# younggyoseo/CaDM

Measured on AMD Instinct MI355X. Metric: CEM rollout row-steps/s (cand x part x horizon x 5 CEM iters per get_action; ens=5 members), higher is better.
Workload: dtype f32 (each fp32 product as 3 f16 MFMA products of 2-way split operands, fp32 accumulate; error <= 2^-22 per product; measured parity: see `parity`); 1 GPU; cfg2: halfcheetah PE-TS+CaDM get_action, ens=5 part=20 cand=200 (200/GPU) H=30 m=1, random-init weights; global_candidates=200, parallelism=candidate-shard x1, collective=none, rccl_nranks=1

## Files before the change

### cadm_amd/csrc/pack_xdl.hip

```cpp
#include "common.h"
#include "xdl_geo.h"

namespace {

struct XdlPackArgs {
    const float* W[CADM_MAX_HIDDEN_LAYERS + 2];
    const float* b[CADM_MAX_HIDDEN_LAYERS + 2];
    unsigned short* dst;
    float* bias;
    int* overflow;
    XdlGeo g;
    int E;
    int swish_fold;
};

__device__ __forceinline__ unsigned short f16_bits(_Float16 h) { return __builtin_bit_cast(unsigned short, h); }

__global__ void pack_xdl_kernel(const XdlPackArgs a) {
    const XdlGeo& g = a.g;
    const size_t per_member = (size_t)g.member_frags() * 1024;
    const size_t total = per_member * a.E;
    for (size_t idx = blockIdx.x * (size_t)blockDim.x + threadIdx.x; idx < total; idx += (size_t)gridDim.x * blockDim.x) {
        const int e = idx / per_member;
        size_t rem = idx % per_member;
        int w = 0;
        while (rem >= (size_t)g.wave_frags(w) * 1024) { rem -= (size_t)g.wave_frags(w) * 1024; ++w; }
        int fj = rem / 1024;
        const int part = (rem % 1024) / 512;
        const int lane = (rem % 512) / 8;
        const int i = rem % 8;
        const int ntw = g.ntw(w);
        int layer, nchl;
        const int nc0s = g.NC0 - g.INV;
        const int inv0 = ntw * nc0s + (g.NH - 1) * ntw * g.NCH + g.nhead(w) * g.NCH;
        bool invf = false;
        if (g.INV && fj >= inv0) { invf = true; layer = 0; nchl = 1; fj -= inv0; }
        else if (fj < ntw * nc0s) { layer = 0; nchl = nc0s; }
        else {
            fj -= ntw * nc0s;
            layer = 1 + fj / (ntw * g.NCH);
            nchl = g.NCH;
            if (layer < g.NH) fj -= (layer - 1) * ntw * g.NCH;
            else { fj -= (g.NH - 1) * ntw * g.NCH; layer = g.NH; }
        }
        const int grp = lane >> 4, m = lane & 15;
        int tile, c;
        if (invf) { tile = g.tstart(w) + fj; c = g.NC0 - 1; }
        else if (layer < g.NH) {
            const int gsz = xdl_group();
            const int gi = fj / (gsz * nchl), jj = fj - gsz * gi * nchl;
            const int gs = (ntw - gsz * gi) < gsz ? (ntw - gsz * gi) : gsz;
            c = jj / gs;
            tile = g.tstart(w) + gsz * gi + jj % gs;
        } else {
            int sv = fj / g.NCH;
            c = fj % g.NCH;
            tile = -1;
            for (int s = 0; s < g.NTOW; ++s) {
                if (g.head_tile(w, s) < g.NTO) { if (sv == 0) { tile = g.head_tile(w, s); break; } --sv; }
            }
        }
        int kin;
        if (layer == 0) { kin = 32 * c + 8 * grp + i; if (kin >= g.K0) kin = -1; }
        else { kin = (2 * c + (i >> 2)) * 16 + 4 * grp + (i & 3); if (kin >= g.HIDR) kin = -1; }
        const int K = layer == 0 ? g.K0 : g.HIDR;
        float v = 0.0f;
        if (kin >= 0 && tile >= 0) {
            if (layer < g.NH) {
                const int u = 16 * tile + m;
                if (u < g.HIDR) v = a.W[layer][((size_t)e * K + kin) * g.HIDR + u];
            } else {
                const int q = m >> 2, r = m & 3;
                const int d = 8 * tile + 2 * q + (r & 1);
                if (d < g.D) v = a.W[g.NH + (r >> 1)][((size_t)e * K + kin) * g.D + d];
            }
        }
        if (a.swish_fold) v *= layer == 0 ? CADM_XDL_LOG2E : layer == g.NH ? (1.0f / CADM_XDL_LOG2E) : 1.0f;
        if (!(fabsf(v) <= 65000.0f)) { *a.overflow = 1; v = 0.0f; }
        const _Float16 v1 = (_Float16)v;
        const _Float16 v2 = (_Float16)((v - (float)v1) * 2048.0f);
        a.dst[idx] = f16_bits(part == 0 ? v1 : v2);
    }
}

__global__ void pack_xdl_bias_kernel(const XdlPackArgs a) {
    const XdlGeo& g = a.g;
    const size_t per = (size_t)g.bias_tiles() * 256;
    const size_t total = per * a.E;
    for (size_t idx = blockIdx.x * (size_t)blockDim.x + threadIdx.x; idx < total; idx += (size_t)gridDim.x * blockDim.x) {
        const int e = idx / per;
        const size_t rem = idx % per;
        int tile = rem / 256;
        const int lane = (rem % 256) / 4, r = rem % 4, grp = lane >> 4;
        float v = 0.0f;
        if (tile < g.NH * g.NT) {
            const int layer = tile / g.NT;
            tile %= g.NT;
            const int u = 16 * tile + 4 * grp + r;
            if (u < g.HIDR) v = a.b[layer][(size_t)e * g.HIDR + u];
            if (a.swish_fold) v *= CADM_XDL_LOG2E;
        } else {
            tile -= g.NH * g.NT;
            const int d = 8 * tile + 2 * grp + (r & 1);
            if (d < g.D) v = a.b[g.NH + (r >> 1)][(size_t)e * g.D + d];
// ... 41 lines not shown
```

### cadm_amd/csrc/rollout_xdl.h

```cpp
#pragma once
#include "rollout_args.h"
#include "rollout_env.h"
#include "xdl_geo.h"

namespace {

typedef _Float16 f16x8 __attribute__((ext_vector_type(8)));
typedef _Float16 f16x4 __attribute__((ext_vector_type(4)));
typedef _Float16 f16x2 __attribute__((ext_vector_type(2)));
typedef float floatx2 __attribute__((ext_vector_type(2)));

template <int ENV_, int C_, int HID_, int MT_, int NH_, int ACT_>
struct XC {
    static constexpr int ENV = ENV_, C = C_, HID = HID_, MT = MT_, NHC = NH_, ACT = ACT_;
    static_assert(NH_ >= 1 && NH_ <= CADM_MAX_HIDDEN_LAYERS, "number of hidden layers");
    static constexpr int D = env_D(ENV), A = env_A(ENV), P = env_P(ENV);
    static constexpr int K0 = P + A + C;
    static constexpr int NC0 = (K0 + 31) / 32;
    static constexpr bool SPARE = (K0 % 32) != 0;
    static constexpr int NT = (HID + 15) / 16;
    static constexpr bool INV = xdl_inv0(K0, P + A, HID);
    static constexpr int NC0S = NC0 - (INV ? 1 : 0);
    static constexpr int NCH = (NT + 1) / 2;
    static constexpr int NTO = (D + 7) / 8;
    static constexpr int NW = CADM_XDL_WAVES, NTHR = NW * 64;
    static constexpr int BASE = NT / NW, EXTRA = NT % NW;
    static constexpr int NTOW = (NTO + NW - 1) / NW;
    static_assert(NTOW == 1, "one head tile per wave at most (obs dim <= 64)");
    static constexpr int R = 4;
    static constexpr int NPROD = HID > 256 ? 4 : 3;
    static constexpr int NP = (D + 1) / 2, NPI = (NP + 15) / 16, NAI = (A + 15) / 16;
    static_assert(BASE >= 1, "hidden width too small for the 8-wave tile split (>= 128)");
    static constexpr int XIN = 0;
    static constexpr int XIN_T = 2 * NC0 * 1024, ACT_T = 2 * NCH * 1024, OFULL_T = NTO * 1024;
    static constexpr int ACTA = XIN + MT * XIN_T;
    static constexpr int ACTB = ACTA + MT * ACT_T;
    static constexpr int OFULL = ACTB + MT * ACT_T;
    static constexpr int STATS = OFULL + MT * OFULL_T;
    static constexpr int ST_OBS_MEAN = 0, ST_OBS_DEN = P, ST_ACT_MEAN = 2 * P, ST_ACT_DEN = 2 * P + A;
    static constexpr int TABW = 28;
    static constexpr int TAB = STATS + rup((2 * P + 2 * A) * 4, 16);
    static constexpr bool ONED = MT == 1 && NPI == 1 && D + NP <= 32 && A <= D;
    static constexpr int TABD = 16;
    static constexpr int TAB_BYTES = ONED ? 32 * TABD * 4 : NPI * 16 * TABW * 4;
    static constexpr int ZB = TAB + TAB_BYTES;
    static constexpr int ZB_T = 2 * NPI * 256 * 8;
    static constexpr int CTRL = ZB + MT * ZB_T;
    static constexpr int RES_1 = 16;
    static constexpr int RES_MT2_LESS = 6;
// ... 41 lines not shown

__device__ __forceinline__ void xres_load(uintx4& dst, __amdgpu_buffer_rsrc_t rsrc, unsigned voff, unsigned soff) {
    asm volatile("s_nop 4\n\tbuffer_load_dwordx4 %0, %1, %2, %3 offen"
                 : "=a"(dst) : "v"(voff), "s"(rsrc), "s"(__builtin_amdgcn_readfirstlane(soff)) : "memory");
}
__device__ __forceinline__ void xmfma_res(floatx4& acc, const uintx4& w, const f16x8& x) {
    asm volatile("s_nop 1\n\tv_mfma_f32_16x16x32_f16 %0, %1, %2, %0" : "+v"(acc) : "a"(w), "v"(x));
}
template <bool ASM>
__device__ __forceinline__ void xmfma_ring(floatx4& acc, const uintx4& w, const f16x8& x) {
    if constexpr (ASM) asm volatile("s_nop 1\n\tv_mfma_f32_16x16x32_f16 %0, %1, %2, %0" : "+v"(acc) : "v"(w), "v"(x));
    else acc = xmfma(w, x, acc);
}
template <bool LL>
__device__ __forceinline__ void xdl_result_nops(floatx4& a, floatx4& b, floatx4& c) {
    if constexpr (LL) asm volatile("s_nop 7\n\ts_nop 7\n\ts_nop 3" : "+v"(a), "+v"(b), "+v"(c));
    else asm volatile("s_nop 7\n\ts_nop 7\n\ts_nop 3" : "+v"(a), "+v"(b));
}
template <bool LL>
__device__ __forceinline__ void xdl_operand_nops(floatx4& a, floatx4& b, floatx4& c) {
    if constexpr (LL) asm volatile("s_nop 4" : "+v"(a), "+v"(b), "+v"(c));
    else asm volatile("s_nop 4" : "+v"(a), "+v"(b));
}

__device__ __forceinline__ void xsplit(float v, _Float16& hi, _Float16& lo) {
    hi = (_Float16)v;
    lo = (_Float16)(v - (float)hi);
}

template <class G, bool PACKED = true>
struct XHiddenEpi {
    static constexpr int NSTAGE = 6;
    struct StateP { floatx2 v[2], s[2]; f16x4 h1, h2; };
    struct StateS { float v[4], s[4]; f16x4 h1, h2; };
    using State = std::conditional_t<PACKED, StateP, StateS>;
    unsigned char* xsmem;
    const float* xb;
    int bias_off;
    int layer, out, tstart, lane;
    const unsigned char* inv = nullptr;
    __device__ __forceinline__ floatx4 init(int ti, int hh) const {
        if (inv) return *reinterpret_cast<const floatx4*>(inv + ((hh * G::NT + tstart + ti) * 2 + 0) * 1024 + lane * 16);
        const int tile = layer * G::NT + tstart + ti;
        const int bt = tile * 64 + lane;
        if constexpr (G::BIAS_LDS) return *reinterpret_cast<const floatx4*>(xsmem + bias_off + tile * G::BIAS_TILE_B + (lane >> 4) * 16);
        else return *reinterpret_cast<const floatx4*>(xb + bt * 4);
    }
    __device__ __forceinline__ floatx4 init_lo(int ti, int hh) const {
        if (inv) return *reinterpret_cast<const floatx4*>(inv + ((hh * G::NT + tstart + ti) * 2 + 1) * 1024 + lane * 16);
        return floatx4{0.f, 0.f, 0.f, 0.f};
    }
    static __device__ __forceinline__ floatx2 lo2(const floatx4& x) { return __builtin_shufflevector(x, x, 0, 1); }
    static __device__ __forceinline__ floatx2 hi2(const floatx4& x) { return __builtin_shufflevector(x, x, 2, 3); }
    template <int S>
    __device__ __forceinline__ void stage(int ti, int hh, const floatx4& hi, const floatx4& lo, const floatx4& ll, State& st) const {
        constexpr float KE = G::ACT == CADM_ACT_TANH ? -2.0f * 1.4426950408889634f : -1.4426950408889634f;
        constexpr bool SIG = G::ACT != CADM_ACT_RELU && G::ACT != CADM_ACT_NONE;
        if constexpr (PACKED) {
        if constexpr (S == 0) {
            const floatx2 c11 = {4.8828125e-4f, 4.8828125e-4f};
            const floatx2 ke = {KE, KE};
#pragma unroll
            for (int q = 0; q < 2; ++q) {
                const floatx2 pre = __builtin_elementwise_fma(q ? hi2(lo) : lo2(lo), c11, q ? hi2(hi) : lo2(hi));
                st.v[q] = pre;
                if constexpr (G::ACT == CADM_ACT_SWISH) st.s[q] = -pre;
                else st.s[q] = pre * ke;
            }
        } else if constexpr (S == 1) {
            if constexpr (SIG) {
#pragma unroll
                for (int q = 0; q < 2; ++q) { st.s[q][0] = __builtin_amdgcn_exp2f(st.s[q][0]); st.s[q][1] = __builtin_amdgcn_exp2f(st.s[q][1]); }
            }
        } else if constexpr (S == 2) {
            if constexpr (SIG) {
                const floatx2 one = {1.0f, 1.0f};
#pragma unroll
                for (int q = 0; q < 2; ++q) {
                    st.s[q] = st.s[q] + one;
                    st.s[q][0] = __builtin_amdgcn_rcpf(st.s[q][0]);
                    st.s[q][1] = __builtin_amdgcn_rcpf(st.s[q][1]);
                }
            }
        } else if constexpr (S == 3) {
#pragma unroll
            for (int q = 0; q < 2; ++q) {
                if constexpr (G::ACT == CADM_ACT_SWISH) st.v[q] = st.v[q] * st.s[q];
                else if constexpr (G::ACT == CADM_ACT_SIGMOID) st.v[q] = st.s[q];
                else if constexpr (G::ACT == CADM_ACT_TANH) {
#pragma unroll
                    for (int r = 0; r < 2; ++r) {
                        const float x = st.v[q][r], x2 = x * x;
                        const float ser = x * fmaf(x2, fmaf(x2, fmaf(x2, -0.05396825396825397f, 0.13333333333333333f), -0.3333333333333333f), 1.0f);
                        st.v[q][r] = fabsf(x) < 0.1f ? ser : fmaf(2.0f, st.s[q][r], -1.0f);
                    }
                } else if constexpr (G::ACT == CADM_ACT_RELU) { st.v[q][0] = fmaxf(st.v[q][0], 0.0f); st.v[q][1] = fmaxf(st.v[q][1], 0.0f); }
                st.h1[2 * q] = (_Float16)st.v[q][0];
                st.h1[2 * q + 1] = (_Float16)st.v[q][1];
            }
        } else if constexpr (S == 4) {
#pragma unroll
            for (int q = 0; q < 2; ++q) {
                const floatx2 t = st.v[q];
                const f16x2 hp = {st.h1[2 * q], st.h1[2 * q + 1]};
                f16x2 lp;
                asm("v_fma_mixlo_f16 %0, %1, %2, %3 op_sel_hi:[1,0,0]\n\tv_fma_mixhi_f16 %0, %1, %2, %4 op_sel:[1,0,0] op_sel_hi:[1,0,0]"
                    : "=&v"(lp) : "v"(hp), "s"(-1.0f), "v"(t[0]), "v"(t[1]));
                st.h2[2 * q] = lp[0];
                st.h2[2 * q + 1] = lp[1];
            }
        }
        } else {
        if constexpr (S == 0) {
#pragma unroll
            for (int r = 0; r < 4; ++r) {
                st.v[r] = fmaf(lo[r], 4.8828125e-4f, hi[r]);
                if constexpr (SIG && G::ACT != CADM_ACT_SWISH) st.s[r] = st.v[r] * KE;
            }
        } else if constexpr (S == 1) {
            if constexpr (SIG) {
#pragma unroll
                for (int r = 0; r < 4; ++r) st.s[r] = __builtin_amdgcn_exp2f(G::ACT == CADM_ACT_SWISH ? -st.v[r] : st.s[r]);
            }
        } else if constexpr (S == 2) {
            if constexpr (SIG) {
// ... 5 lines not shown
            for (int r = 0; r < 4; ++r) {
                if constexpr (G::ACT == CADM_ACT_SWISH) st.v[r] = st.v[r] * st.s[r];
                else if constexpr (G::ACT == CADM_ACT_SIGMOID) st.v[r] = st.s[r];
                else if constexpr (G::ACT == CADM_ACT_TANH) {
                    const float x = st.v[r], x2 = x * x;
                    const float ser = x * fmaf(x2, fmaf(x2, fmaf(x2, -0.05396825396825397f, 0.13333333333333333f), -0.3333333333333333f), 1.0f);
                    st.v[r] = fabsf(x) < 0.1f ? ser : fmaf(2.0f, st.s[r], -1.0f);
                } else if constexpr (G::ACT == CADM_ACT_RELU) st.v[r] = fmaxf(st.v[r], 0.0f);
                st.h1[r] = (_Float16)st.v[r];
            }
        } else if constexpr (S == 4) {
#pragma unroll
            for (int q = 0; q < 2; ++q) {
                const f16x2 hp = {st.h1[2 * q], st.h1[2 * q + 1]};
                f16x2 lp;
                asm("v_fma_mixlo_f16 %0, %1, %2, %3 op_sel_hi:[1,0,0]\n\tv_fma_mixhi_f16 %0, %1, %2, %4 op_sel:[1,0,0] op_sel_hi:[1,0,0]"
                    : "=&v"(lp) : "v"(hp), "s"(-1.0f), "v"(st.v[2 * q]), "v"(st.v[2 * q + 1]));
                st.h2[2 * q] = lp[0];
                st.h2[2 * q + 1] = lp[1];
            }
        }
        }
        if constexpr (S == 5) {
            const int Tg = tstart + ti;
            unsigned char* dst = xsmem + out + hh * G::ACT_T + ((Tg >> 1) * 64 + lane) * 16 + (Tg & 1) * 8;
            *reinterpret_cast<f16x4*>(dst) = st.h1;
            *reinterpret_cast<f16x4*>(dst + G::NCH * 1024) = st.h2;
        }
    }
};

template <class G>
struct XHeadEpi {
    static constexpr int NSTAGE = 1;
    struct State {};
    unsigned char* xsmem;
    const float* xb;
    int bias_off, bias_tile, ht, lane;
    __device__ __forceinline__ floatx4 init_lo(int, int) const { return floatx4{0.f, 0.f, 0.f, 0.f}; }
    __device__ __forceinline__ floatx4 init(int, int) const {
        const int bt = bias_tile * 64 + lane;
        if constexpr (G::BIAS_LDS) return *reinterpret_cast<const floatx4*>(xsmem + bias_off + bias_tile * G::BIAS_TILE_B + (lane >> 4) * 16);
        else return *reinterpret_cast<const floatx4*>(xb + bt * 4);
    }
    template <int S>
    __device__ __forceinline__ void stage(int, int hh, const floatx4& hi, const floatx4& lo, const floatx4& ll, State&) const {
        floatx4 v;
#pragma unroll
        for (int r = 0; r < 4; ++r) {
            v[r] = fmaf(lo[r], 4.8828125e-4f, hi[r]);
        }
        *reinterpret_cast<floatx4*>(xsmem + G::OFULL + hh * G::OFULL_T + (ht * 64 + lane) * 16) = v;
    }
};

template <class G, int NTW, int NCHL, int NRES, int GS, bool SIDE, int NLDS, int NCB = NCHL, class Epi>
__device__ __forceinline__ void xdl_sweep(XRing<G>& ring, const uintx4 (*res)[2], __amdgpu_buffer_rsrc_t rsrc, unsigned wcur,
                                          unsigned wnext, int nx_nf, const unsigned char* lds_in, int lane, const Epi& epi,
                                          const unsigned char* lq TS_PARAMS) {
    constexpr int R = G::R, NF = NTW * NCHL, NFS = NF - NRES, NFSPAD = rup(NFS, R);
    static_assert(NRES >= 0 && NRES <= NF, "bad resident fragment count");
    static_assert(NLDS == 0 || NFS - NLDS >= R, "the first R ring fragments of a layer are streamed");
    constexpr int MT = G::MT, XD = NCHL < G::XDEPTH ? NCHL : G::XDEPTH;
    constexpr int IN_T = 2 * NCB * 1024;
    f16x8 X1[XD][MT], X2[XD][MT];
    auto xload = [&](auto cc) {
        constexpr int c = decltype(cc)::value;
#pragma unroll
        for (int h = 0; h < MT; ++h) {
            X1[c % XD][h] = *reinterpret_cast<const f16x8*>(lds_in + h * IN_T + ((0 * NCB + c) * 64 + lane) * 16);
            X2[c % XD][h] = *reinterpret_cast<const f16x8*>(lds_in + h * IN_T + ((1 * NCB + c) * 64 + lane) * 16);
        }
    };
    auto prefetch = [&](auto jsc) {
        constexpr int js = decltype(jsc)::value;
        constexpr int jj = js + R;
        if constexpr (jj < NFS - NLDS) {
            xring_load<js % R>(ring, rsrc, wcur + jj * CADM_XDL_FRAG_BYTES, lane);
        } else if constexpr (jj < NFS) {
            const unsigned char* p = lq + (jj - (NFS - NLDS)) * CADM_XDL_FRAG_BYTES + lane * 16;
            ring.w[js % R][0] = *reinterpret_cast<const uintx4*>(p);
            ring.w[js % R][1] = *reinterpret_cast<const uintx4*>(p + 1024);
        } else if constexpr (jj >= NFSPAD) {
            if (jj - NFSPAD < nx_nf) xring_load<js % R>(ring, rsrc, wnext + (jj - NFSPAD) * CADM_XDL_FRAG_BYTES, lane);
        }
    };
    constexpr int NG = (NTW + GS - 1) / GS, NST = Epi::NSTAGE;
    constexpr int NPR = G::NPROD;
    floatx4 hi[2][GS][MT], lo[2][GS][MT], ll[2][GS][MT];
    typename Epi::State pst[GS][MT];
    auto stage_chunk = [](int st) constexpr { return NCHL == 1 ? 0 : NST == 1 ? 1 : 1 + st * (NCHL - 2) / (NST - 1); };
    TR_DECL
    TR(0)
    static_for(std::make_integer_sequence<int, NG>{}, [&](auto gc) {
        constexpr int g = decltype(gc)::value, gp = g & 1, pp = gp ^ 1;
        constexpr int gs = (NTW - GS * g) < GS ? (NTW - GS * g) : GS;
        constexpr int pgs = (SIDE && g > 0) ? GS : 0;
        static_for(std::make_integer_sequence<int, XD - 1>{}, [&](auto cc) { xload(cc); });
#pragma unroll
        for (int k = 0; k < gs; ++k)
#pragma unroll
            for (int h = 0; h < MT; ++h) {
                hi[gp][k][h] = epi.init(GS * g + k, h); lo[gp][k][h] = epi.init_lo(GS * g + k, h); ll[gp][k][h] = floatx4{0.f, 0.f, 0.f, 0.f};
            }
#pragma unroll
        for (int k = 0; k < gs; ++k)
#pragma unroll
            for (int h = 0; h < MT; ++h) xdl_operand_nops<false>(hi[gp][k][h], lo[gp][k][h], ll[gp][k][h]);
        static_for(std::make_integer_sequence<int, NCHL>{}, [&](auto cc) {
            constexpr int c = decltype(cc)::value;
            constexpr int j0 = GS * g * NCHL + c * gs;
            if constexpr (c == 1 && g == 0) { TS(10) }
            if constexpr (c + XD - 1 < NCHL) xload(std::integral_constant<int, c + XD - 1>{});
            static_for(std::make_integer_sequence<int, NPR * gs * MT>{}, [&](auto mc) {
                constexpr int h = decltype(mc)::value % MT, k = (decltype(mc)::value / MT) % gs, prod = decltype(mc)::value / (MT * gs);
                constexpr int j = j0 + k;
                floatx4& acc = (prod == 0 || prod == 2) ? hi[gp][k][h] : lo[gp][k][h];
                const f16x8& x = prod >= 2 ? X2[c % XD][h] : X1[c % XD][h];
                constexpr int part = (prod == 1 || prod == 3) ? 1 : 0;
                if constexpr (j < NRES) xmfma_res(acc, res[j][part], x);
                else xmfma_ring<G::ASM_MFMA>(acc, ring.w[(j - NRES) % R][part], x);
            });
            static_for(std::make_integer_sequence<int, gs>{}, [&](auto kc) {
                constexpr int j = j0 + decltype(kc)::value;
                if constexpr (j >= NRES) prefetch(std::integral_constant<int, j - NRES>{});
            });
            if constexpr (pgs > 0) {
                static_for(std::make_integer_sequence<int, NST>{}, [&](auto sc) {
                    constexpr int st = decltype(sc)::value;
                    if constexpr (stage_chunk(st) == c) {
#pragma unroll
                        for (int k = 0; k < pgs; ++k)
#pragma unroll
                            for (int h = 0; h < MT; ++h)
                                epi.template stage<st>(GS * (g - 1) + k, h, hi[pp][k][h], lo[pp][k][h], ll[pp][k][h], pst[k][h]);
                    }
                });
            }
            if constexpr (g == NG - 1 && c < 8) { TR(1 + c) }
            __builtin_amdgcn_sched_barrier(0);
        });
        if constexpr (g == NG - 1 || !SIDE) {
            TS(11)
#pragma unroll
            for (int k = 0; k < gs; ++k)
#pragma unroll
                for (int h = 0; h < MT; ++h) xdl_result_nops<false>(hi[gp][k][h], lo[gp][k][h], ll[gp][k][h]);
            static_for(std::make_integer_sequence<int, NST>{}, [&](auto sc) {
#pragma unroll
                for (int k = 0; k < gs; ++k)
#pragma unroll
                    for (int h = 0; h < MT; ++h)
                        epi.template stage<decltype(sc)::value>(GS * g + k, h, hi[gp][k][h], lo[gp][k][h], ll[gp][k][h], pst[k][h]);
            });
        }
    });
    TS(12)
    TR(10)
    TR_FLUSH
    static_for(std::make_integer_sequence<int, NFSPAD - NFS>{}, [&](auto jc) {
        prefetch(std::integral_constant<int, NFS + decltype(jc)::value>{});
    });
}

template <class G, int NOISE, int NTW>
__device__ __forceinline__ void xdl_run(const RolloutArgs& a, unsigned char* xsmem) {
    constexpr int D = G::D, A = G::A, P = G::P, C = G::C, K0 = G::K0, NC0 = G::NC0, NCH = G::NCH, NTO = G::NTO;
    constexpr int NP = G::NP, NPI = G::NPI, NAI = G::NAI, ENV = G::ENV, R = G::R;
    constexpr int MT = G::MT;
    constexpr int XNH = G::NHC;
    const int tid = threadIdx.x;
    const int lane = tid & 63;
    const int wave = __builtin_amdgcn_readfirstlane(tid >> 6);
    const int item = rollout_item();
    const int e = item / a.wgs_per_member;
    const int grp = item % a.wgs_per_member;
    const int H = a.H;
    const bool need_last = a.traj != nullptr || ENV == CADM_ENV_CARTPOLE || has_next<ENV>();
    const int t_end = need_last ? H : H - 1;
    const int arow = tid & 15, fg = (tid >> 4) & 15;
    constexpr bool ONED = G::ONED;
    const int sd = tid >> 4;
    const bool feat = ONED ? sd < D : (MT > 1 || wave < 4);
    const bool nzt = ONED && sd >= 32 - NP;
    const bool actt = ONED && sd >= 32 - A;
    const int rt = MT > 1 ? (wave >> 2) : 0;
    const int ntiles = a.tile_count;
    float* stats = reinterpret_cast<float*>(xsmem + G::STATS);
    float* ctrl_s = reinterpret_cast<float*>(xsmem + G::CTRL) + rt * 16 * H;
// ... 66 lines not shown
                    te[10 + 2 * h + i] = a.obs_mean[f];
                    te[14 + 2 * h + i] = 1.0f / (a.obs_std[f] + 1e-10f);
                    te[18 + 2 * h + i] = __builtin_bit_cast(float, on ? xin_base(f) : -1);
                    te[22 + 2 * h + i] = __builtin_bit_cast(float, on ? fop[i] : 0);
                }
            }
        }
    }
    const int a0 = (fg - (NP & 15) + 16) & 15;
    float ret = 0.0f;
    auto put_x = [&](int off, float v) {
        ret = fmaf(0.0f, v, ret);
        asm volatile("" : "+v"(v));
        _Float16 h1, h2;
        xsplit(v, h1, h2);
        *reinterpret_cast<_Float16*>(xsmem + xin_rt + off) = h1;
        *reinterpret_cast<_Float16*>(xsmem + xin_rt + NC0 * 1024 + off) = h2;
    };

    const __amdgpu_buffer_rsrc_t rsrc = __builtin_amdgcn_make_buffer_rsrc((void*)a.xw, 0, a.xw_bytes, 0x00020000);
    const unsigned wbase = e * a.xw_member_b + a.xw_wave_b[wave];
    const float* xb = a.xb + (size_t)e * a.xb_member;
    const int my_ntw = G::BASE + (wave < G::EXTRA ? 1 : 0);
    const int tstart = wave * G::BASE + (wave < G::EXTRA ? wave : G::EXTRA);
    const int ht = G::NW - 1 - wave;
    const int nhead = ht < NTO ? 1 : 0;
    const int l0_nf = my_ntw * G::NC0S, lh_nf = my_ntw * NCH, hd_nf = nhead * NCH;
    const unsigned w_l0 = wbase, w_h1 = w_l0 + l0_nf * CADM_XDL_FRAG_BYTES;
    const unsigned w_hd = w_h1 + (XNH - 1) * lh_nf * CADM_XDL_FRAG_BYTES;
    const unsigned w_inv = w_hd + hd_nf * CADM_XDL_FRAG_BYTES;
    const int inv_off = bias_off + (G::BIAS_LDS ? G::BIAS_BYTES : 0) + G::LQ_BYTES;

    constexpr int GSZ = xdl_group();
    constexpr int NFH = NTW * NCH;
    constexpr bool RESO = NTW == G::BASE && G::res_frags(NTW) >= NCH + 3;
    constexpr int RREM = G::res_frags(NTW) - (RESO ? NCH : 0);
    constexpr int Q1 = cmin((RREM + 2) / 3, NFH), Q2 = cmin((RREM - Q1 + 1) / 2, NFH), Q3 = cmin(RREM - Q1 - Q2, NFH);
    constexpr int NRESH = Q1 + Q2 + Q3;
    auto hq = [&](int l) { return l == 1 ? Q1 : l == 2 ? Q2 : l == 3 ? Q3 : 0; };
    auto lay_res = [&](int l) { return l == 0 ? 0 : l < XNH ? hq(l) : RESO ? hd_nf : 0; };
    auto lay_off = [&](int l) {
        return (l == 0 ? w_l0 : l < XNH ? w_h1 + (l - 1) * lh_nf * CADM_XDL_FRAG_BYTES : w_hd) + lay_res(l) * CADM_XDL_FRAG_BYTES;
    };
    auto lay_nf = [&](int l) { return (l == 0 ? l0_nf : l < XNH ? lh_nf : hd_nf) - lay_res(l); };
    auto next_streamed = [&](int l) {
        for (int k = 0; k <= XNH; ++k) {
            l = l == XNH ? 0 : l + 1;
// ... 104 lines not shown
        auto gen_noise = [&](int t) {
#pragma unroll
            for (int pi = 0; pi < NPI; ++pi) {
                const int dp = ONED ? sd - (32 - NP) : fg + 16 * pi;
                if (dp >= NP) continue;
                float2 z;
                if constexpr (NOISE == CADM_NOISE_INJECT) {
                    const float* epp = a.eps + ((size_t)t * a.m * a.n_local * a.p + lr) * D + 2 * dp;
                    z.x = epp[0];
                    z.y = (2 * dp + 1 < D) ? epp[1] : 0.0f;
                } else {
                    uint32_t pc[4] = {grow, (uint32_t)t, eps_group(dp), CADM_STREAM_EPS | ((uint32_t)a.it << 8)};
                    uint32_t pk[2] = {a.seed, a.call};
                    philox_rounds<0, 10>(pc, pk);
                    const bool hi = eps_sub(dp) != 0;
                    box_muller(u01(hi ? pc[2] : pc[0]), u01(hi ? pc[3] : pc[1]), z.x, z.y);
                }
                zb[((t & 1) * NPI + pi) * 256 + (dp & 15) * 16 + arow] = z;
            }
        };
        __syncthreads();
        if constexpr (G::INV) {
            floatx4 ll0 = floatx4{0.f, 0.f, 0.f, 0.f};
            const XHiddenEpi<G> epib{xsmem, xb, bias_off, 0, 0, tstart, lane};
            static_for(std::make_integer_sequence<int, NTW>{}, [&](auto tc) {
                constexpr int ti = decltype(tc)::value;
                const uintx4 w0 = __builtin_amdgcn_raw_buffer_load_b128(rsrc, lane * 16, w_inv + ti * CADM_XDL_FRAG_BYTES, 0);
                const uintx4 w1 = __builtin_amdgcn_raw_buffer_load_b128(rsrc, lane * 16 + 1024, w_inv + ti * CADM_XDL_FRAG_BYTES, 0);
#pragma unroll
                for (int h = 0; h < MT; ++h) {
                    const unsigned char* xin = xsmem + G::XIN + h * G::XIN_T;
                    const f16x8 x1 = *reinterpret_cast<const f16x8*>(xin + ((0 * NC0 + NC0 - 1) * 64 + lane) * 16);
                    const f16x8 x2 = *reinterpret_cast<const f16x8*>(xin + ((1 * NC0 + NC0 - 1) * 64 + lane) * 16);
                    floatx4 hi = epib.init(ti, h), lo = floatx4{0.f, 0.f, 0.f, 0.f};
                    xdl_operand_nops<false>(hi, lo, ll0);
                    xmfma_ring<G::ASM_MFMA>(hi, w0, x1);
                    xmfma_ring<G::ASM_MFMA>(lo, w1, x1);
                    xmfma_ring<G::ASM_MFMA>(hi, w0, x2);
                    xdl_result_nops<false>(hi, lo, ll0);
                    unsigned char* dst = xsmem + inv_off + ((h * G::NT + tstart + ti) * 2) * 1024 + lane * 16;
                    *reinterpret_cast<floatx4*>(dst) = hi;
                    *reinterpret_cast<floatx4*>(dst + 1024) = lo;
                }
            });
        }
        TS_DECL

        for (int t = 0; t <= H; ++t) {
            if constexpr (ONED) {
                const int dp = sd >> 1, hh = sd & 1;
                if (feat) {
                    floatx4 tq[4];
#pragma unroll
                    for (int q = 0; q < 4; ++q) tq[q] = *reinterpret_cast<const floatx4*>(tab + sd * G::TABD + 4 * q);
                    auto tv = [&](int w) { return tq[w >> 2][w & 3]; };
                    auto ti_ = [&](int w) { const float fv = tq[w >> 2][w & 3]; return __float_as_int(fv); };
                    if (t > 0) {
                        const int jt = dp >> 2, lt = (dp & 3) * 16 + arow;
                        const float* vp = ofull + (jt * 64 + lt) * 4;
                        float delta = vp[hh] * tv(1) + tv(0);
                        if constexpr (NOISE != CADM_NOISE_NONE) {
                            const float z = reinterpret_cast<const float*>(zb + ((t - 1) & 1) * 256 + dp * 16 + arow)[hh];
                            const float sdv = head_sd(vp[2 + hh], tv(3), tv(4), tv(2));
                            delta = delta + z * sdv;
                        }
// ... 88 lines not shown
            if (t < H) {
#pragma unroll
                for (int ai = 0; ai < NAI; ++ai) {
                    const int ac = a0 + 16 * ai;
                    if (ac < A) {
                        float v = areg[ai];
                        if (a.norm_actions) v = (v - stats[G::ST_ACT_MEAN + ac]) * stats[G::ST_ACT_DEN + ac];
                        put_x(xin_off(P + ac), v);
                        if (t + 1 < H) areg[ai] = a.actions[abase + (t + 1) * A + ac];
                    }
                }
            }
            }
            if (t >= t_end) break;
            if constexpr (NOISE != CADM_NOISE_NONE && MT == 1) {
                if (ONED ? nzt : !feat) gen_noise(t);
            }
            TS(0)
            __syncthreads();
            TS(1)

            {
                int act_out = G::ACTA, act_in = G::XIN;
                auto hidden_epi = [&](int layer, int out) { return XHiddenEpi<G>{xsmem, xb, bias_off, layer, out, tstart, lane}; };
                {
                    const int nx = next_streamed(0);
                    XHiddenEpi<G> epi0 = hidden_epi(0, act_out);
                    if constexpr (G::INV) epi0.inv = xsmem + inv_off;
                    xdl_sweep<G, NTW, G::NC0S, 0, GSZ, true, 0, NC0>(ring, nullptr, rsrc, w_l0, lay_off(nx), lay_nf(nx), xsmem + act_in, lane,
                                              epi0, nullptr TS_ARGS);
                }
                TS(2)
                __syncthreads();
                TS(3)
                if constexpr (ONED && XNH == 1) {
                    if (actt && t + 1 < H) act_put(t + 1);
                }
                auto hidden = [&](int l, auto res_c, auto base_c, auto lq_c) {
                    constexpr int NRES = decltype(res_c)::value, RBASE = decltype(base_c)::value;
                    act_in = act_out;
                    act_out = (act_in == G::ACTA) ? G::ACTB : G::ACTA;
                    const int nx = next_streamed(l);
                    constexpr int NL = decltype(lq_c)::value ? LQ : 0;
                    TR_ON(t == 10 && l == 2, wave)
                    xdl_sweep<G, NTW, NCH, NRES, GSZ, true, NL>(ring, resH + RBASE, rsrc, lay_off(l), lay_off(nx), lay_nf(nx), xsmem + act_in, lane,
                                                 hidden_epi(l, act_out), xsmem + lq_off + (l - 1) * LQ * CADM_XDL_FRAG_BYTES TS_ARGS);
                    if constexpr (NOISE != CADM_NOISE_NONE && MT > 1) {
                        if (l == 1 && nhead) gen_noise(t);
                    }
                    if constexpr (ONED) {
                        if (l == 1 && actt && t + 1 < H) act_put(t + 1);
                    }
                    if (l == 1) { TS(4) } else if (l == 2) { TS(8) } else { TS(9) }
                    __syncthreads();
                    TR_LATE(11)
                    TR_ON(false, 0)
                    TS(5)
                };
                using IC0 = std::integral_constant<int, 0>;
                using IC1 = std::integral_constant<int, 1>;
                if (1 < XNH) hidden(1, std::integral_constant<int, Q1>{}, IC0{}, IC1{});
                if (2 < XNH) hidden(2, std::integral_constant<int, Q2>{}, std::integral_constant<int, Q1>{}, IC1{});
                if (3 < XNH) hidden(3, std::integral_constant<int, Q3>{}, std::integral_constant<int, Q1 + Q2>{}, IC1{});
                for (int l = 4; l < XNH; ++l) hidden(l, IC0{}, IC0{}, IC0{});
                act_in = act_out;
                if constexpr (NOISE != CADM_NOISE_NONE && MT > 1) {
                    if (!nhead || XNH < 2) gen_noise(t);
                }
// ... 26 lines not shown
            if (feat) ret_s[arow * 16 + fg] = ret;
            ret = 0.0f;
            __syncthreads();
            if (feat && fg == 0 && valid) {
                float r = 0.0f;
#pragma unroll
                for (int i = 0; i < 16; ++i) r += ret_s[arow * 16 + i];
                a.returns_rows[lr] = r;
            }
        }
        __syncthreads();
    }
}

template <class G, int NOISE>
__global__ __launch_bounds__(G::NTHR) void rollout_xdl_kernel(const RolloutArgs a) {
    extern __shared__ __attribute__((aligned(16))) unsigned char xsmem_raw[];
    fp16_saturate_on();
    const int wave = __builtin_amdgcn_readfirstlane(threadIdx.x >> 6);
    if constexpr (G::MT > 1) {
        if (wave >= G::NW / 2) __builtin_amdgcn_s_setprio(1);
    }
    if (wave < G::EXTRA) {
        if constexpr (G::EXTRA > 0) xdl_run<G, NOISE, G::BASE + 1>(a, xsmem_raw);
    } else {
        xdl_run<G, NOISE, G::BASE>(a, xsmem_raw);
    }
}

template <class G, int NOISE>
int xdl_launch_noise(cadm_ctx* ctx, const RolloutArgs& a, int rows_per_member, hipStream_t s) {
    RolloutArgs args = a;
    const int tiles = (a.tile_count + G::MT - 1) / G::MT;
    int per_member = ctx->n_cus / ctx->E;
    if (per_member < 1) per_member = 1;
    args.wgs_per_member = tiles < per_member ? tiles : per_member;
    args.rows_per_member = rows_per_member;
    const size_t lds = G::lds_bytes(a.H);
    args.bias_lds = G::BIAS_LDS;
    if (lds > 160 * 1024) {
        cadm_set_error("rollout: horizon %d with %d hidden layers of %d units needs %zu B of LDS (> 160 KiB)", a.H, G::NHC, G::HID, lds);
        return CADM_EINVAL;
    }
    const void* fn = reinterpret_cast<const void*>(&rollout_xdl_kernel<G, NOISE>);
    if (!ctx->attr_done.count(fn)) {
        CADM_CHECK_HIP(hipFuncSetAttribute(fn, hipFuncAttributeMaxDynamicSharedMemorySize, 160 * 1024));
        ctx->attr_done.insert(fn);
    }
    if (a.dry_run) return CADM_OK;
// ... 78 lines not shown
```

### cadm_amd/csrc/xdl_geo.h

```cpp
#pragma once

#define CADM_XDL_FRAG_BYTES 2048
#define CADM_XDL_LOG2E 1.4426950408889634f
#define CADM_XDL_WAVES 8

#define CADM_XDL_MIN_HID 113
#define CADM_XDL_NARROW_HID 128
__host__ __device__ constexpr int xdl_kernel_hid(int hid) { return hid < CADM_XDL_MIN_HID ? CADM_XDL_NARROW_HID : hid; }

__host__ __device__ constexpr bool xdl_inv0(int k0, int kdyn, int hid_kernel) {
    return k0 > kdyn && (k0 + 31) / 32 >= 2 && ((k0 + 31) / 32 - 1) * 32 >= kdyn && (hid_kernel + 15) / 16 <= 13;
}

struct XdlGeo {
    int K0, HID, D, NH, HIDR;
    int INV;
    int NC0, NT, NCH, NTO, BASE, EXTRA, NTOW;
    int NW;
    __host__ __device__ int ntw(int w) const { return BASE + (w < EXTRA ? 1 : 0); }
    __host__ __device__ int tstart(int w) const { return w * BASE + (w < EXTRA ? w : EXTRA); }
    __host__ __device__ int head_tile(int w, int s) const { return (NW - 1 - w) + NW * s; }
    __host__ __device__ int nhead(int w) const {
        int n = 0;
        for (int s = 0; s < NTOW; ++s) n += head_tile(w, s) < NTO ? 1 : 0;
        return n;
    }
    __host__ __device__ int wave_frags(int w) const { return ntw(w) * NC0 + (NH - 1) * ntw(w) * NCH + nhead(w) * NCH; }
    __host__ __device__ int member_frags() const {
        int n = 0;
        for (int w = 0; w < NW; ++w) n += wave_frags(w);
        return n;
    }
    __host__ __device__ int bias_tiles() const { return NH * NT + NTO; }
};

inline XdlGeo make_xdl_geo(int K0, int hid_model, int D, int NH, int nw = CADM_XDL_WAVES, int kdyn = -1) {
    XdlGeo g;
    g.NW = nw;
    g.INV = (nw == CADM_XDL_WAVES && kdyn >= 0 && xdl_inv0(K0, kdyn, xdl_kernel_hid(hid_model))) ? 1 : 0;
    const int HID = xdl_kernel_hid(hid_model);
    g.K0 = K0; g.HID = HID; g.HIDR = hid_model; g.D = D; g.NH = NH;
    g.NC0 = (K0 + 31) / 32;
    g.NT = (HID + 15) / 16;
    g.NCH = (g.NT + 1) / 2;
    g.NTO = (D + 7) / 8;
    g.BASE = g.NT / nw;
    g.EXTRA = g.NT % nw;
    g.NTOW = (g.NTO + nw - 1) / nw;
    return g;
}

__host__ __device__ constexpr int xdl_group() { return 2; }

__host__ __device__ constexpr int xdl_frag_index(int ntw, int nchl, int ti, int c, int gsz) {
    const int g = ti / gsz;
    const int gs = (ntw - gsz * g) < gsz ? (ntw - gsz * g) : gsz;
    return gsz * g * nchl + c * gs + (ti - gsz * g);
}

struct XdlCosts { float c[4]; float wt8p[3]; };
__host__ __device__ constexpr XdlCosts xdl_costs(int env_kind, int hid) {
    return env_kind == 2  ? XdlCosts{{1.0f, 1.62f, 3.62f, 5.5f}, {4.78f, 4.80f, 5.15f}}
                                                      : XdlCosts{{1.0f, 1.59f, 3.2f, 5.19f}, {4.48f, 4.52f, 4.84f}};
}
inline void xdl_plan_units(int units, bool mt2_ok, bool wt_ok, int (&count)[4], XdlCosts costs = xdl_costs(0, 200)) {
    const int capu[4] = {1, mt2_ok ? 2 : 0, wt_ok ? 4 : 0, wt_ok ? 8 : 0};
    const float* cost = costs.c;
    for (int o = 0; o < 4; ++o) count[o] = 0;
    const int big = capu[3] ? 3 : capu[1] ? 1 : 0;
    int u = units;
    if (u > 64) { const int k = (u - 56) / capu[big]; count[big] += k; u -= k * capu[big]; }
// ... 16 lines not shown
```

Baseline: 796.9 million row-steps/s.

## Use two-product half-tile MFMA for the partial last hidden tile

When the hidden width leaves a last 16-wide tile at most half full (HID=200, 13 tiles), that tile's hi and lo weight splits are packed into the two halves of one fragment. The tile then needs only two MFMA products instead of three and a single accumulator, with a permlane32 swap to separate the halves in the epilogue. Ownership of that tile moves to a wave with fewer tiles to rebalance load. This removes wasted MFMA work on zero-padded columns but adds a lane swap, special-case epilogue stores and extra template instantiations that may raise register use or code size.

```diff
diff --git a/cadm_amd/csrc/pack_xdl.hip b/cadm_amd/csrc/pack_xdl.hip
--- a/cadm_amd/csrc/pack_xdl.hip
+++ b/cadm_amd/csrc/pack_xdl.hip
@@ -45,13 +45,13 @@
         }
         const int grp = lane >> 4, m = lane & 15;
         int tile, c;
-        if (invf) { tile = g.tstart(w) + fj; c = g.NC0 - 1; }
+        if (invf) { tile = g.tile_of(w, fj); c = g.NC0 - 1; }
         else if (layer < g.NH) {
             const int gsz = xdl_group();
             const int gi = fj / (gsz * nchl), jj = fj - gsz * gi * nchl;
             const int gs = (ntw - gsz * gi) < gsz ? (ntw - gsz * gi) : gsz;
             c = jj / gs;
-            tile = g.tstart(w) + gsz * gi + jj % gs;
+            tile = g.tile_of(w, gsz * gi + jj % gs);
         } else {
             int sv = fj / g.NCH;
             c = fj % g.NCH;
@@ -64,11 +64,12 @@
         if (layer == 0) { kin = 32 * c + 8 * grp + i; if (kin >= g.K0) kin = -1; }
         else { kin = (2 * c + (i >> 2)) * 16 + 4 * grp + (i & 3); if (kin >= g.HIDR) kin = -1; }
         const int K = layer == 0 ? g.K0 : g.HIDR;
+        const bool half = g.HALF && layer < g.NH && tile == g.NT - 1;
         float v = 0.0f;
         if (kin >= 0 && tile >= 0) {
             if (layer < g.NH) {
-                const int u = 16 * tile + m;
-                if (u < g.HIDR) v = a.W[layer][((size_t)e * K + kin) * g.HIDR + u];
+                const int u = 16 * tile + (half ? (m & 7) : m);
+                if (u < g.HIDR && !(half && part == 1 && m >= 8)) v = a.W[layer][((size_t)e * K + kin) * g.HIDR + u];
             } else {
                 const int q = m >> 2, r = m & 3;
                 const int d = 8 * tile + 2 * q + (r & 1);
@@ -79,7 +80,7 @@
         if (!(fabsf(v) <= 65000.0f)) { *a.overflow = 1; v = 0.0f; }
         const _Float16 v1 = (_Float16)v;
         const _Float16 v2 = (_Float16)((v - (float)v1) * 2048.0f);
-        a.dst[idx] = f16_bits(part == 0 ? v1 : v2);
+        a.dst[idx] = f16_bits(half ? (m < 8 ? v1 : v2) : part == 0 ? v1 : v2);
     }
 }
 
diff --git a/cadm_amd/csrc/rollout_xdl.h b/cadm_amd/csrc/rollout_xdl.h
--- a/cadm_amd/csrc/rollout_xdl.h
+++ b/cadm_amd/csrc/rollout_xdl.h
@@ -25,6 +25,9 @@
     static constexpr int NTO = (D + 7) / 8;
     static constexpr int NW = CADM_XDL_WAVES, NTHR = NW * 64;
     static constexpr int BASE = NT / NW, EXTRA = NT % NW;
+    static constexpr bool HALF = xdl_half(HID, NW), MOVED = xdl_half_moved(HID, NW);
+    static constexpr int HALFW = xdl_half_wave(HID, NW);
+    static_assert(xdl_owners_ok(HID, NW), "hidden tile ownership: every tile exactly one owner");
     static constexpr int NTOW = (NTO + NW - 1) / NW;
     static_assert(NTOW == 1, "one head tile per wave at most (obs dim <= 64)");
     static constexpr int R = 4;
@@ -112,13 +115,25 @@
     if constexpr (LL) asm volatile("s_nop 4" : "+v"(a), "+v"(b), "+v"(c));
     else asm volatile("s_nop 4" : "+v"(a), "+v"(b));
 }
+__device__ __forceinline__ void xdl_result_nops1(floatx4& a) { asm volatile("s_nop 7\n\ts_nop 7\n\ts_nop 3" : "+v"(a)); }
+__device__ __forceinline__ void xdl_operand_nops1(floatx4& a) { asm volatile("s_nop 4" : "+v"(a)); }
+__device__ __forceinline__ void xdl_half_pairs(const floatx4& acc, floatx2& hp, floatx2& lp) {
+#pragma unroll
+    for (int k = 0; k < 2; ++k) {
+        const float fa = acc[2 * k], fb = acc[2 * k + 1];
+        const auto s = __builtin_amdgcn_permlane32_swap(__float_as_uint(fa), __float_as_uint(fb), false, false);
+        const unsigned ua = s[0], ub = s[1];
+        hp[k] = __uint_as_float(ua);
+        lp[k] = __uint_as_float(ub);
+    }
+}
 
 __device__ __forceinline__ void xsplit(float v, _Float16& hi, _Float16& lo) {
     hi = (_Float16)v;
     lo = (_Float16)(v - (float)hi);
 }
 
-template <class G, bool PACKED = true>
+template <class G, bool PACKED = true, int HT = -1>
 struct XHiddenEpi {
     static constexpr int NSTAGE = 6;
     struct StateP { floatx2 v[2], s[2]; f16x4 h1, h2; };
@@ -129,30 +144,37 @@
     int bias_off;
     int layer, out, tstart, lane;
     const unsigned char* inv = nullptr;
+    __device__ __forceinline__ int gtile(int ti) const { return (HT >= 0 && ti == HT) ? G::NT - 1 : tstart + ti; }
     __device__ __forceinline__ floatx4 init(int ti, int hh) const {
-        if (inv) return *reinterpret_cast<const floatx4*>(inv + ((hh * G::NT + tstart + ti) * 2 + 0) * 1024 + lane * 16);
-        const int tile = layer * G::NT + tstart + ti;
+        if (inv) return *reinterpret_cast<const floatx4*>(inv + ((hh * G::NT + gtile(ti)) * 2 + 0) * 1024 + lane * 16);
+        const int tile = layer * G::NT + gtile(ti);
         const int bt = tile * 64 + lane;
         if constexpr (G::BIAS_LDS) return *reinterpret_cast<const floatx4*>(xsmem + bias_off + tile * G::BIAS_TILE_B + (lane >> 4) * 16);
         else return *reinterpret_cast<const floatx4*>(xb + bt * 4);
     }
     __device__ __forceinline__ floatx4 init_lo(int ti, int hh) const {
-        if (inv) return *reinterpret_cast<const floatx4*>(inv + ((hh * G::NT + tstart + ti) * 2 + 1) * 1024 + lane * 16);
+        if (inv) return *reinterpret_cast<const floatx4*>(inv + ((hh * G::NT + gtile(ti)) * 2 + 1) * 1024 + lane * 16);
         return floatx4{0.f, 0.f, 0.f, 0.f};
     }
     static __device__ __forceinline__ floatx2 lo2(const floatx4& x) { return __builtin_shufflevector(x, x, 0, 1); }
     static __device__ __forceinline__ floatx2 hi2(const floatx4& x) { return __builtin_shufflevector(x, x, 2, 3); }
     template <int S>
-    __device__ __forceinline__ void stage(int ti, int hh, const floatx4& hi, const floatx4& lo, const floatx4& ll, State& st) const {
+    __device__ __forceinline__ void stage(int ti, int hh, const floatx4& hi, const floatx4& lo_, const floatx4& ll, State& st) const {
+        const floatx4& lo = lo_;
+        const bool half = HT >= 0 && ti == HT;
+        const int nq = half ? 1 : 2;
         constexpr float KE = G::ACT == CADM_ACT_TANH ? -2.0f * 1.4426950408889634f : -1.4426950408889634f;
         constexpr bool SIG = G::ACT != CADM_ACT_RELU && G::ACT != CADM_ACT_NONE;
         if constexpr (PACKED) {
         if constexpr (S == 0) {
             const floatx2 c11 = {4.8828125e-4f, 4.8828125e-4f};
             const floatx2 ke = {KE, KE};
+            floatx2 hp = lo2(hi), lp = lo2(lo);
+            if (half) xdl_half_pairs(hi, hp, lp);
 #pragma unroll
             for (int q = 0; q < 2; ++q) {
-                const floatx2 pre = __builtin_elementwise_fma(q ? hi2(lo) : lo2(lo), c11, q ? hi2(hi) : lo2(hi));
+                if (q >= nq) continue;
+                const floatx2 pre = __builtin_elementwise_fma(q ? hi2(lo) : lp, c11, q ? hi2(hi) : hp);
                 st.v[q] = pre;
                 if constexpr (G::ACT == CADM_ACT_SWISH) st.s[q] = -pre;
                 else st.s[q] = pre * ke;
@@ -160,13 +182,14 @@
         } else if constexpr (S == 1) {
             if constexpr (SIG) {
 #pragma unroll
-                for (int q = 0; q < 2; ++q) { st.s[q][0] = __builtin_amdgcn_exp2f(st.s[q][0]); st.s[q][1] = __builtin_amdgcn_exp2f(st.s[q][1]); }
+                for (int q = 0; q < 2; ++q) { if (q >= nq) continue; st.s[q][0] = __builtin_amdgcn_exp2f(st.s[q][0]); st.s[q][1] = __builtin_amdgcn_exp2f(st.s[q][1]); }
             }
         } else if constexpr (S == 2) {
             if constexpr (SIG) {
                 const floatx2 one = {1.0f, 1.0f};
 #pragma unroll
                 for (int q = 0; q < 2; ++q) {
+                    if (q >= nq) continue;
                     st.s[q] = st.s[q] + one;
                     st.s[q][0] = __builtin_amdgcn_rcpf(st.s[q][0]);
                     st.s[q][1] = __builtin_amdgcn_rcpf(st.s[q][1]);
@@ -175,6 +198,7 @@
         } else if constexpr (S == 3) {
 #pragma unroll
             for (int q = 0; q < 2; ++q) {
+                if (q >= nq) continue;
                 if constexpr (G::ACT == CADM_ACT_SWISH) st.v[q] = st.v[q] * st.s[q];
                 else if constexpr (G::ACT == CADM_ACT_SIGMOID) st.v[q] = st.s[q];
                 else if constexpr (G::ACT == CADM_ACT_TANH) {
@@ -191,6 +215,7 @@
         } else if constexpr (S == 4) {
 #pragma unroll
             for (int q = 0; q < 2; ++q) {
+                if (q >= nq) continue;
                 const floatx2 t = st.v[q];
                 const f16x2 hp = {st.h1[2 * q], st.h1[2 * q + 1]};
                 f16x2 lp;
@@ -242,10 +267,18 @@
         }
         }
         if constexpr (S == 5) {
-            const int Tg = tstart + ti;
+            const int Tg = gtile(ti);
             unsigned char* dst = xsmem + out + hh * G::ACT_T + ((Tg >> 1) * 64 + lane) * 16 + (Tg & 1) * 8;
-            *reinterpret_cast<f16x4*>(dst) = st.h1;
-            *reinterpret_cast<f16x4*>(dst + G::NCH * 1024) = st.h2;
+            if (half) {
+                unsigned char* d2 = xsmem + out + hh * G::ACT_T + ((Tg >> 1) * 64 + (lane & 31)) * 16 + (Tg & 1) * 8 + (lane >> 5) * 2;
+                *reinterpret_cast<_Float16*>(d2) = st.h1[0];
+                *reinterpret_cast<_Float16*>(d2 + 4) = st.h1[1];
+                *reinterpret_cast<_Float16*>(d2 + G::NCH * 1024) = st.h2[0];
+                *reinterpret_cast<_Float16*>(d2 + G::NCH * 1024 + 4) = st.h2[1];
+            } else {
+                *reinterpret_cast<f16x4*>(dst) = st.h1;
+                *reinterpret_cast<f16x4*>(dst + G::NCH * 1024) = st.h2;
+            }
         }
     }
 };
@@ -274,7 +307,7 @@
     }
 };
 
-template <class G, int NTW, int NCHL, int NRES, int GS, bool SIDE, int NLDS, int NCB = NCHL, class Epi>
+template <class G, int NTW, int NCHL, int NRES, int GS, bool SIDE, int NLDS, int NCB = NCHL, int HT = -1, class Epi>
 __device__ __forceinline__ void xdl_sweep(XRing<G>& ring, const uintx4 (*res)[2], __amdgpu_buffer_rsrc_t rsrc, unsigned wcur,
                                           unsigned wnext, int nx_nf, const unsigned char* lds_in, int lane, const Epi& epi,
                                           const unsigned char* lq TS_PARAMS) {
@@ -306,6 +339,7 @@
         }
     };
     constexpr int NG = (NTW + GS - 1) / GS, NST = Epi::NSTAGE;
+    static_assert(HT < 0 || (HT == NTW - 1 && G::NPROD == 3 && G::ASM_MFMA), "the half tile is the wave's last tile; three products per block");
     constexpr int NPR = G::NPROD;
     floatx4 hi[2][GS][MT], lo[2][GS][MT], ll[2][GS][MT];
     typename Epi::State pst[GS][MT];
@@ -326,7 +360,10 @@
 #pragma unroll
         for (int k = 0; k < gs; ++k)
 #pragma unroll
-            for (int h = 0; h < MT; ++h) xdl_operand_nops<false>(hi[gp][k][h], lo[gp][k][h], ll[gp][k][h]);
+            for (int h = 0; h < MT; ++h) {
+                if (HT >= 0 && GS * g + k == HT) xdl_operand_nops1(hi[gp][k][h]);
+                else xdl_operand_nops<false>(hi[gp][k][h], lo[gp][k][h], ll[gp][k][h]);
+            }
         static_for(std::make_integer_sequence<int, NCHL>{}, [&](auto cc) {
             constexpr int c = decltype(cc)::value;
             constexpr int j0 = GS * g * NCHL + c * gs;
@@ -335,10 +372,12 @@
             static_for(std::make_integer_sequence<int, NPR * gs * MT>{}, [&](auto mc) {
                 constexpr int h = decltype(mc)::value % MT, k = (decltype(mc)::value / MT) % gs, prod = decltype(mc)::value / (MT * gs);
                 constexpr int j = j0 + k;
+                constexpr bool half = HT >= 0 && GS * g + k == HT;
                 floatx4& acc = (prod == 0 || prod == 2) ? hi[gp][k][h] : lo[gp][k][h];
                 const f16x8& x = prod >= 2 ? X2[c % XD][h] : X1[c % XD][h];
-                constexpr int part = (prod == 1 || prod == 3) ? 1 : 0;
-                if constexpr (j < NRES) xmfma_res(acc, res[j][part], x);
+                constexpr int part = half ? (prod == 2 ? 1 : 0) : (prod == 1 || prod == 3) ? 1 : 0;
+                if constexpr (half && prod == 1) {}
+                else if constexpr (j < NRES) xmfma_res(acc, res[j][part], x);
                 else xmfma_ring<G::ASM_MFMA>(acc, ring.w[(j - NRES) % R][part], x);
             });
             static_for(std::make_integer_sequence<int, gs>{}, [&](auto kc) {
@@ -365,7 +404,10 @@
 #pragma unroll
             for (int k = 0; k < gs; ++k)
 #pragma unroll
-                for (int h = 0; h < MT; ++h) xdl_result_nops<false>(hi[gp][k][h], lo[gp][k][h], ll[gp][k][h]);
+                for (int h = 0; h < MT; ++h) {
+                    if (HT >= 0 && GS * g + k == HT) xdl_result_nops1(hi[gp][k][h]);
+                    else xdl_result_nops<false>(hi[gp][k][h], lo[gp][k][h], ll[gp][k][h]);
+                }
             static_for(std::make_integer_sequence<int, NST>{}, [&](auto sc) {
 #pragma unroll
                 for (int k = 0; k < gs; ++k)
@@ -383,8 +425,10 @@
     });
 }
 
-template <class G, int NOISE, int NTW>
+template <class G, int NOISE, int NTW, bool HALFB = false>
 __device__ __forceinline__ void xdl_run(const RolloutArgs& a, unsigned char* xsmem) {
+    constexpr int HT = HALFB ? NTW - 1 : -1;
+    using HEpi = XHiddenEpi<G, true, HT>;
     constexpr int D = G::D, A = G::A, P = G::P, C = G::C, K0 = G::K0, NC0 = G::NC0, NCH = G::NCH, NTO = G::NTO;
     constexpr int NP = G::NP, NPI = G::NPI, NAI = G::NAI, ENV = G::ENV, R = G::R;
     constexpr int MT = G::MT;
@@ -497,7 +541,7 @@
     const unsigned wbase = e * a.xw_member_b + a.xw_wave_b[wave];
     const float* xb = a.xb + (size_t)e * a.xb_member;
     const int my_ntw = G::BASE + (wave < G::EXTRA ? 1 : 0);
-    const int tstart = wave * G::BASE + (wave < G::EXTRA ? wave : G::EXTRA);
+    const int tstart = G::MOVED ? wave * G::BASE + (wave < G::EXTRA - 1 ? wave : G::EXTRA - 1) : wave * G::BASE + (wave < G::EXTRA ? wave : G::EXTRA);
     const int ht = G::NW - 1 - wave;
     const int nhead = ht < NTO ? 1 : 0;
     const int l0_nf = my_ntw * G::NC0S, lh_nf = my_ntw * NCH, hd_nf = nhead * NCH;
@@ -648,7 +692,7 @@
         __syncthreads();
         if constexpr (G::INV) {
             floatx4 ll0 = floatx4{0.f, 0.f, 0.f, 0.f};
-            const XHiddenEpi<G> epib{xsmem, xb, bias_off, 0, 0, tstart, lane};
+            const HEpi epib{xsmem, xb, bias_off, 0, 0, tstart, lane};
             static_for(std::make_integer_sequence<int, NTW>{}, [&](auto tc) {
                 constexpr int ti = decltype(tc)::value;
                 const uintx4 w0 = __builtin_amdgcn_raw_buffer_load_b128(rsrc, lane * 16, w_inv + ti * CADM_XDL_FRAG_BYTES, 0);
@@ -659,14 +703,22 @@
                     const f16x8 x1 = *reinterpret_cast<const f16x8*>(xin + ((0 * NC0 + NC0 - 1) * 64 + lane) * 16);
                     const f16x8 x2 = *reinterpret_cast<const f16x8*>(xin + ((1 * NC0 + NC0 - 1) * 64 + lane) * 16);
                     floatx4 hi = epib.init(ti, h), lo = floatx4{0.f, 0.f, 0.f, 0.f};
-                    xdl_operand_nops<false>(hi, lo, ll0);
-                    xmfma_ring<G::ASM_MFMA>(hi, w0, x1);
-                    xmfma_ring<G::ASM_MFMA>(lo, w1, x1);
-                    xmfma_ring<G::ASM_MFMA>(hi, w0, x2);
-                    xdl_result_nops<false>(hi, lo, ll0);
-                    unsigned char* dst = xsmem + inv_off + ((h * G::NT + tstart + ti) * 2) * 1024 + lane * 16;
-                    *reinterpret_cast<floatx4*>(dst) = hi;
-                    *reinterpret_cast<floatx4*>(dst + 1024) = lo;
+                    unsigned char* dst = xsmem + inv_off + ((h * G::NT + epib.gtile(ti)) * 2) * 1024 + lane * 16;
+                    if constexpr (ti == HT) {
+                        xdl_operand_nops1(hi);
+                        xmfma_ring<G::ASM_MFMA>(hi, w0, x1);
+                        xmfma_ring<G::ASM_MFMA>(hi, w1, x2);
+                        xdl_result_nops1(hi);
+                        *reinterpret_cast<floatx4*>(dst) = hi;
+                    } else {
+                        xdl_operand_nops<false>(hi, lo, ll0);
+                        xmfma_ring<G::ASM_MFMA>(hi, w0, x1);
+                        xmfma_ring<G::ASM_MFMA>(lo, w1, x1);
+                        xmfma_ring<G::ASM_MFMA>(hi, w0, x2);
+                        xdl_result_nops<false>(hi, lo, ll0);
+                        *reinterpret_cast<floatx4*>(dst) = hi;
+                        *reinterpret_cast<floatx4*>(dst + 1024) = lo;
+                    }
                 }
             });
         }
@@ -801,12 +853,12 @@
 
             {
                 int act_out = G::ACTA, act_in = G::XIN;
-                auto hidden_epi = [&](int layer, int out) { return XHiddenEpi<G>{xsmem, xb, bias_off, layer, out, tstart, lane}; };
+                auto hidden_epi = [&](int layer, int out) { return HEpi{xsmem, xb, bias_off, layer, out, tstart, lane}; };
                 {
                     const int nx = next_streamed(0);
-                    XHiddenEpi<G> epi0 = hidden_epi(0, act_out);
+                    HEpi epi0 = hidden_epi(0, act_out);
                     if constexpr (G::INV) epi0.inv = xsmem + inv_off;
-                    xdl_sweep<G, NTW, G::NC0S, 0, GSZ, true, 0, NC0>(ring, nullptr, rsrc, w_l0, lay_off(nx), lay_nf(nx), xsmem + act_in, lane,
+                    xdl_sweep<G, NTW, G::NC0S, 0, GSZ, true, 0, NC0, HT>(ring, nullptr, rsrc, w_l0, lay_off(nx), lay_nf(nx), xsmem + act_in, lane,
                                               epi0, nullptr TS_ARGS);
                 }
                 TS(2)
@@ -822,7 +874,7 @@
                     const int nx = next_streamed(l);
                     constexpr int NL = decltype(lq_c)::value ? LQ : 0;
                     TR_ON(t == 10 && l == 2, wave)
-                    xdl_sweep<G, NTW, NCH, NRES, GSZ, true, NL>(ring, resH + RBASE, rsrc, lay_off(l), lay_off(nx), lay_nf(nx), xsmem + act_in, lane,
+                    xdl_sweep<G, NTW, NCH, NRES, GSZ, true, NL, NCH, HT>(ring, resH + RBASE, rsrc, lay_off(l), lay_off(nx), lay_nf(nx), xsmem + act_in, lane,
                                                  hidden_epi(l, act_out), xsmem + lq_off + (l - 1) * LQ * CADM_XDL_FRAG_BYTES TS_ARGS);
                     if constexpr (NOISE != CADM_NOISE_NONE && MT > 1) {
                         if (l == 1 && nhead) gen_noise(t);
@@ -895,9 +947,17 @@
         if (wave >= G::NW / 2) __builtin_amdgcn_s_setprio(1);
     }
     if (wave < G::EXTRA) {
-        if constexpr (G::EXTRA > 0) xdl_run<G, NOISE, G::BASE + 1>(a, xsmem_raw);
+        if constexpr (G::EXTRA > 0) {
+            if constexpr (G::HALF && G::HALFW < G::EXTRA) {
+                if (wave == G::HALFW) xdl_run<G, NOISE, G::BASE + 1, true>(a, xsmem_raw);
+                else if constexpr (G::EXTRA > 1) xdl_run<G, NOISE, G::BASE + 1>(a, xsmem_raw);
+            } else xdl_run<G, NOISE, G::BASE + 1>(a, xsmem_raw);
+        }
     } else {
-        xdl_run<G, NOISE, G::BASE>(a, xsmem_raw);
+        if constexpr (G::HALF && G::HALFW >= G::EXTRA) {
+            if (wave == G::HALFW) xdl_run<G, NOISE, G::BASE, true>(a, xsmem_raw);
+            else xdl_run<G, NOISE, G::BASE>(a, xsmem_raw);
+        } else xdl_run<G, NOISE, G::BASE>(a, xsmem_raw);
     }
 }
 
diff --git a/cadm_amd/csrc/xdl_geo.h b/cadm_amd/csrc/xdl_geo.h
--- a/cadm_amd/csrc/xdl_geo.h
+++ b/cadm_amd/csrc/xdl_geo.h
@@ -8,6 +8,38 @@
 #define CADM_XDL_NARROW_HID 128
 __host__ __device__ constexpr int xdl_kernel_hid(int hid) { return hid < CADM_XDL_MIN_HID ? CADM_XDL_NARROW_HID : hid; }
 
+__host__ __device__ constexpr bool xdl_half(int hid_kernel, int nw) {
+    return nw == CADM_XDL_WAVES && hid_kernel <= 256 && hid_kernel % 16 >= 1 && hid_kernel % 16 <= 8;
+}
+__host__ __device__ constexpr bool xdl_half_moved(int hid_kernel, int nw) {
+    return xdl_half(hid_kernel, nw) && (((hid_kernel + 15) / 16) % nw) % 4 == 1;
+}
+__host__ __device__ constexpr int xdl_half_wave(int hid_kernel, int nw) {
+    return !xdl_half(hid_kernel, nw) ? -1 : xdl_half_moved(hid_kernel, nw) ? ((hid_kernel + 15) / 16) % nw - 1 : nw - 1;
+}
+__host__ __device__ constexpr int xdl_tile_of(int nt, int nw, bool moved, int w, int ti) {
+    const int base = nt / nw, extra = nt % nw;
+    if (!moved) return w * base + (w < extra ? w : extra) + ti;
+    if (w == extra - 1 && ti == base) return nt - 1;
+    return w * base + (w < extra - 1 ? w : extra - 1) + ti;
+}
+__host__ __device__ constexpr bool xdl_owners_ok(int hid_kernel, int nw) {
+    const int nt = (hid_kernel + 15) / 16, base = nt / nw, extra = nt % nw;
+    for (int t = 0; t < nt; ++t) {
+        int n = 0;
+        for (int w = 0; w < nw; ++w)
+            for (int ti = 0; ti < base + (w < extra ? 1 : 0); ++ti) n += xdl_tile_of(nt, nw, xdl_half_moved(hid_kernel, nw), w, ti) == t ? 1 : 0;
+        if (n != 1) return false;
+    }
+    const int hw = xdl_half_wave(hid_kernel, nw);
+    return hw < 0 || xdl_tile_of(nt, nw, xdl_half_moved(hid_kernel, nw), hw, base + (hw < extra ? 1 : 0) - 1) == nt - 1;
+}
+static_assert(xdl_owners_ok(128, CADM_XDL_WAVES) && xdl_owners_ok(200, CADM_XDL_WAVES) && xdl_owners_ok(256, CADM_XDL_WAVES) &&
+              xdl_owners_ok(512, CADM_XDL_WAVES) && xdl_owners_ok(200, 1), "hidden tile ownership: every tile exactly one owner");
+static_assert(!xdl_half(128, CADM_XDL_WAVES) && xdl_half(200, CADM_XDL_WAVES) && !xdl_half(256, CADM_XDL_WAVES) && !xdl_half(512, CADM_XDL_WAVES) &&
+              xdl_half_wave(200, CADM_XDL_WAVES) == 4 && xdl_tile_of(13, CADM_XDL_WAVES, true, 4, 1) == 12 && xdl_tile_of(13, CADM_XDL_WAVES, true, 7, 0) == 11 &&
+              xdl_half_wave(120, CADM_XDL_WAVES) == 7 && xdl_half_wave(196, CADM_XDL_WAVES) == 4, "half tile: of the compiled-in widths only 200");
+
 __host__ __device__ constexpr bool xdl_inv0(int k0, int kdyn, int hid_kernel) {
     return k0 > kdyn && (k0 + 31) / 32 >= 2 && ((k0 + 31) / 32 - 1) * 32 >= kdyn && (hid_kernel + 15) / 16 <= 13;
 }
@@ -17,8 +49,10 @@
     int INV;
     int NC0, NT, NCH, NTO, BASE, EXTRA, NTOW;
     int NW;
+    int HALF;
+    int HALFW;
     __host__ __device__ int ntw(int w) const { return BASE + (w < EXTRA ? 1 : 0); }
-    __host__ __device__ int tstart(int w) const { return w * BASE + (w < EXTRA ? w : EXTRA); }
+    __host__ __device__ int tile_of(int w, int ti) const { return xdl_tile_of(NT, NW, HALF && xdl_half_moved(HID, NW), w, ti); }
     __host__ __device__ int head_tile(int w, int s) const { return (NW - 1 - w) + NW * s; }
     __host__ __device__ int nhead(int w) const {
         int n = 0;
@@ -47,6 +81,8 @@
     g.BASE = g.NT / nw;
     g.EXTRA = g.NT % nw;
     g.NTOW = (g.NTO + nw - 1) / nw;
+    g.HALF = xdl_half(HID, nw) ? 1 : 0;
+    g.HALFW = xdl_half_wave(HID, nw);
     return g;
 }
 
```

New measurement: 809.8 million row-steps/s, median of 6. +1.6%, better.
